# amathislab/myochallenge

Measured on AMD Instinct MI355X. Metric: env-steps/sec (Baoding, 4096 envs), higher is better.
Workload: dtype f64

## Files before the change

### myochallenge_amd/csrc/myo_ppo_mlp.h

```cpp
#pragma once
#ifndef MYO_EMU
#include "myo_act.h"

typedef __attribute__((ext_vector_type(8))) __bf16 myo_bf16x8;
typedef __attribute__((ext_vector_type(4))) float myo_f32x4;

#define MLP_H 256
#define MLP_OPMAX 128
#define MLP_APM 48
#define MLP_AKP 64
#define MLP_XS (MLP_OPMAX + 8)
#define MLP_HS (MLP_H + 8)
#define MLP_DS (MLP_AKP + 8)
#define MLP_SOS 49
#define MLP_SPLITK 16

struct MlpImages { unsigned short *W1p, *W2, *W2T, *Whp, *WhT; float* bias; };
static inline MlpImages mlp_images_carve(unsigned char* base, int OP, size_t* bytes) {
  size_t o = 0;
  auto take = [&](size_t n) { unsigned char* p = base ? base + o : nullptr; o += (n + 255) / 256 * 256; return p; };
  const size_t H = MLP_H;
  MlpImages w;
  w.W1p = (unsigned short*)take(2 * H * OP * 2); w.W2 = (unsigned short*)take(2 * H * H * 2); w.W2T = (unsigned short*)take(2 * H * H * 2);
  w.Whp = (unsigned short*)take(2 * MLP_APM * H * 2); w.WhT = (unsigned short*)take(2 * H * MLP_AKP * 2);
// ... 114 lines not shown
  if (t == 0) { part[3 * blockIdx.x] = (float)n; part[3 * blockIdx.x + 1] = mean; part[3 * blockIdx.x + 2] = (red[0] + red[1]) + (red[2] + red[3]); }
}
__global__ void __launch_bounds__(256) k_adv_merge(const float* __restrict__ part_all, int nb, int B, float* __restrict__ stats) {
  __shared__ float sp[3 * MLP_ADV_BLOCKS];
  const int t = threadIdx.x;
  if (t < 3 * nb) sp[t] = part_all[(size_t)blockIdx.x * 3 * nb + t];
  __syncthreads();
  if (t == 0) mlp_adv_merge(sp, nb, B, stats + 2 * blockIdx.x);
}

struct MlpImgTarget {
  MlpImages img;
  int off_W1[2], off_b1[2], off_W2[2], off_b2[2], off_Wh[2], off_bh[2];
  int O, OP, A;
};
__device__ __forceinline__ void mlp_img_store(const MlpImgTarget& T, int i, float x) {
  constexpr unsigned H = MLP_H;
#pragma unroll
  for (int net = 0; net < 2; ++net) {
    const unsigned Ah = net == 0 ? (unsigned)T.A : 1u;
    unsigned j = (unsigned)(i - T.off_W2[net]);
    if (j < H * H) {
      const unsigned short v = mlp_f2bf(x);
      T.img.W2[net * H * H + j] = v;
      T.img.W2T[net * H * H + (j % H) * H + j / H] = v;
      return;
    }
    j = (unsigned)(i - T.off_W1[net]);
    if (j < H * (unsigned)T.O) { const unsigned o = j / (unsigned)T.O; T.img.W1p[net * H * T.OP + o * T.OP + (j - o * T.O)] = mlp_f2bf(x); return; }
    j = (unsigned)(i - T.off_Wh[net]);
    if (j < Ah * H) {
      const unsigned short v = mlp_f2bf(x);
      T.img.Whp[net * MLP_APM * H + j] = v;
      T.img.WhT[net * H * MLP_AKP + (j % H) * MLP_AKP + j / H] = v;
      return;
    }
    j = (unsigned)(i - T.off_b1[net]);
    if (j < H) { T.img.bias[net * H + j] = x; return; }
    j = (unsigned)(i - T.off_b2[net]);
    if (j < H) { T.img.bias[2 * H + net * H + j] = x; return; }
    j = (unsigned)(i - T.off_bh[net]);
    if (j < Ah) { T.img.bias[4 * H + net * MLP_APM + j] = x; return; }
  }
}

template <int KSTEPS>
__device__ __forceinline__ void mlp_load_w(myo_bf16x8 (&bw)[8][4], const unsigned short* Wg, int w_stride, int n0, int lm, int lq) {
#pragma unroll
  for (int ks = 0; ks < KSTEPS; ++ks)
#pragma unroll
    for (int nt = 0; nt < 4; ++nt) bw[ks][nt] = *reinterpret_cast<const myo_bf16x8*>(Wg + (size_t)(n0 + 16 * nt + lm) * w_stride + 32 * ks + 8 * lq);
  __builtin_amdgcn_sched_barrier(0);
}
template <int KSTEPS, int MT>
__device__ __forceinline__ void mlp_mma_slab(myo_f32x4 (&acc)[MT][4], const unsigned short* As, int as_stride, const myo_bf16x8 (&bw)[8][4],
                                             int lm, int lq) {
#pragma unroll
  for (int mt = 0; mt < MT; ++mt)
#pragma unroll
    for (int nt = 0; nt < 4; ++nt) acc[mt][nt] = myo_f32x4{0.f, 0.f, 0.f, 0.f};
#pragma unroll
  for (int ks = 0; ks < KSTEPS; ++ks) {
#pragma unroll
    for (int m2 = 0; m2 < MT; m2 += 2) {
      myo_bf16x8 a[2];
#pragma unroll
      for (int mt = 0; mt < 2; ++mt) a[mt] = *reinterpret_cast<const myo_bf16x8*>(As + (16 * (m2 + mt) + lm) * as_stride + 32 * ks + 8 * lq);
#pragma unroll
      for (int mt = 0; mt < 2; ++mt)
#pragma unroll
        for (int nt = 0; nt < 4; ++nt) acc[m2 + mt][nt] = __builtin_amdgcn_mfma_f32_16x16x32_bf16(a[mt], bw[ks][nt], acc[m2 + mt][nt], 0, 0, 0);
    }
  }
  __builtin_amdgcn_sched_barrier(0);
}

#ifdef MLP_PROF
__device__ unsigned long long g_mlp_prof[16];
#ifndef MLP_PROF_NET
#define MLP_PROF_NET 0
#endif
#define MLP_STAMP(k) { __syncthreads(); if (threadIdx.x == 0 && blockIdx.x == 3 && blockIdx.y == MLP_PROF_NET) g_mlp_prof[k] = wall_clock64(); }
extern "C" int myo_debug_mlp_prof(unsigned long long* out) { return (int)hipMemcpyFromSymbol(out, HIP_SYMBOL(g_mlp_prof), sizeof g_mlp_prof); }
#else
#define MLP_STAMP(k)
#endif

#ifndef MLP_BM
#define MLP_BM 32
#endif
#define MLP_FWDBWD_LDS (512 + MLP_BM * MLP_XS * 2 + MLP_BM * MLP_HS * 2 + MLP_BM * MLP_SOS * 4 + MLP_BM * MLP_DS * 2 + 128 * 4 + 192 * 4)

template <int ACT>
__device__ __forceinline__ float mlp_act(float x) { return ACT == MYO_ACT_TANH ? myo_act_tanh(x) : fmaxf(x, 0.f); }

template <int MT>
__device__ __forceinline__ void mlp_store_act_tanh(const myo_f32x4 (&acc)[MT][4], const float (&bb)[4], unsigned short* Hs, unsigned short* HT,
                                                   size_t B, int r0, int n0, int lm, int lq) {
#pragma unroll
  for (int mt = 0; mt < MT; ++mt)
#pragma unroll
    for (int nt = 0; nt < 4; ++nt) {
      const int n = n0 + 16 * nt + lm, m = 16 * mt + 4 * lq;
      unsigned short h[4];
#pragma unroll
      for (int r = 0; r < 4; ++r) { h[r] = mlp_f2bf(mlp_act<MYO_ACT_TANH>(acc[mt][nt][r] + bb[nt])); Hs[(m + r) * MLP_HS + n] = h[r]; }
      *reinterpret_cast<uint2*>(HT + (size_t)n * B + r0 + m) = make_uint2((unsigned)h[0] | ((unsigned)h[1] << 16), (unsigned)h[2] | ((unsigned)h[3] << 16));
    }
}
template <int MT>
__device__ __forceinline__ void mlp_load_act(uint2 (&hv)[MT][4], const unsigned short* HT, size_t B, int r0, int n0, int lm, int lq) {
#pragma unroll
  for (int mt = 0; mt < MT; ++mt)
#pragma unroll
    for (int nt = 0; nt < 4; ++nt) hv[mt][nt] = *reinterpret_cast<const uint2*>(HT + (size_t)(n0 + 16 * nt + lm) * B + r0 + 16 * mt + 4 * lq);
  __builtin_amdgcn_sched_barrier(0);
}
template <int MT, bool TO_LDS>
__device__ __forceinline__ void mlp_store_grad_tanh(const myo_f32x4 (&acc)[MT][4], const uint2 (&hv)[MT][4], unsigned short* Hs, unsigned short* HT,
                                                    size_t B, int r0, int n0, int lm, int lq) {
#pragma unroll
  for (int mt = 0; mt < MT; ++mt)
#pragma unroll
    for (int nt = 0; nt < 4; ++nt) {
      const int n = n0 + 16 * nt + lm, m = 16 * mt + 4 * lq;
      const float hf[4] = {__uint_as_float(hv[mt][nt].x << 16), __uint_as_float(hv[mt][nt].x & 0xffff0000u),
                           __uint_as_float(hv[mt][nt].y << 16), __uint_as_float(hv[mt][nt].y & 0xffff0000u)};
      unsigned short h[4];
#pragma unroll
      for (int r = 0; r < 4; ++r) {
        h[r] = mlp_f2bf(mlp_bf2f(mlp_f2bf(acc[mt][nt][r])) * fmaf(-hf[r], hf[r], 1.f));
        if (TO_LDS) Hs[(m + r) * MLP_HS + n] = h[r];
      }
      *reinterpret_cast<uint2*>(HT + (size_t)n * B + r0 + m) = make_uint2((unsigned)h[0] | ((unsigned)h[1] << 16), (unsigned)h[2] | ((unsigned)h[3] << 16));
    }
}

template <int MT>
__device__ __forceinline__ unsigned long long mlp_store_act(const myo_f32x4 (&acc)[MT][4], const float (&bb)[4], unsigned short* Hs, unsigned short* HT,
                                                            size_t B, int r0, int n0, int lm, int lq) {
  static_assert(MT * 16 <= 64, "one mask bit per accumulator element");
  unsigned long long mask = 0;
#pragma unroll
  for (int mt = 0; mt < MT; ++mt)
#pragma unroll
    for (int nt = 0; nt < 4; ++nt) {
      const int n = n0 + 16 * nt + lm, m = 16 * mt + 4 * lq;
      unsigned short h[4];
#pragma unroll
      for (int r = 0; r < 4; ++r) {
        h[r] = mlp_f2bf(fmaxf(acc[mt][nt][r] + bb[nt], 0.f)); Hs[(m + r) * MLP_HS + n] = h[r];
        mask |= (unsigned long long)(h[r] != 0) << (16 * mt + 4 * nt + r);
      }
      *reinterpret_cast<uint2*>(HT + (size_t)n * B + r0 + m) = make_uint2((unsigned)h[0] | ((unsigned)h[1] << 16), (unsigned)h[2] | ((unsigned)h[3] << 16));
    }
  return mask;
}
template <int MT, bool TO_LDS>
__device__ __forceinline__ void mlp_store_grad(const myo_f32x4 (&acc)[MT][4], unsigned long long mask, unsigned short* Hs, unsigned short* HT, size_t B,
                                               int r0, int n0, int lm, int lq) {
#pragma unroll
  for (int mt = 0; mt < MT; ++mt)
#pragma unroll
    for (int nt = 0; nt < 4; ++nt) {
      const int n = n0 + 16 * nt + lm, m = 16 * mt + 4 * lq;
      unsigned short h[4];
#pragma unroll
      for (int r = 0; r < 4; ++r) {
        const unsigned short on = (unsigned short)(-(int)((mask >> (16 * mt + 4 * nt + r)) & 1ull));
        h[r] = mlp_f2bf(acc[mt][nt][r]) & on;
        if (TO_LDS) Hs[(m + r) * MLP_HS + n] = h[r];
      }
      *reinterpret_cast<uint2*>(HT + (size_t)n * B + r0 + m) = make_uint2((unsigned)h[0] | ((unsigned)h[1] << 16), (unsigned)h[2] | ((unsigned)h[3] << 16));
    }
}

template <int ACT>
__global__ void __launch_bounds__(256, 2) k_mlp_fwdbwd(MlpArgs P) {
  constexpr int H = MLP_H, XS = MLP_XS, HS = MLP_HS, DS = MLP_DS, SOS = MLP_SOS, BM = MLP_BM, MT = BM / 16, RW = BM / 4;
  extern __shared__ __align__(16) unsigned char mlp_smem[];
  long long* s_idx = reinterpret_cast<long long*>(mlp_smem);
  unsigned short* Xs = reinterpret_cast<unsigned short*>(mlp_smem + 512);
  float* So = reinterpret_cast<float*>(mlp_smem + 512);
  unsigned short* Hs = Xs + BM * XS;
  float* Sa = reinterpret_cast<float*>(Hs + BM * HS);
  unsigned short* dOs = reinterpret_cast<unsigned short*>(Sa + BM * SOS);
  float* s_ls = reinterpret_cast<float*>(dOs + BM * DS);
  float* s_row = s_ls + 128;
  static_assert(BM * MLP_SOS * 4 <= BM * MLP_XS * 2, "the head output tile fits where X was");
  static_assert(BM == 32 || BM == 64, "wave / tile mapping below");
  const int t = threadIdx.x, w = t >> 6, lane = t & 63, lm = lane & 15, lq = lane >> 4;
  const int net = blockIdx.y, blk = blockIdx.x, r0 = blk * BM, B = P.B, O = P.O, A = P.A, OP = P.OP;
  const int n0 = 64 * w;
  MLP_STAMP(0)
  if (t < BM) s_idx[t] = P.idx[r0 + t];
  if (t < A) { const float ls = P.log_std[t]; s_ls[t] = ls; s_ls[64 + t] = __expf(-ls); }
  const float* b1 = P.img.bias + net * H; const float* b2 = P.img.bias + 2 * H + net * H; const float* bh = P.img.bias + 4 * H + net * MLP_APM;
  float bb1[4], bb2[4];
#pragma unroll
  for (int nt = 0; nt < 4; ++nt) { bb1[nt] = b1[n0 + 16 * nt + lm]; bb2[nt] = b2[n0 + 16 * nt + lm]; }
  myo_bf16x8 bw[8][4];
  {
    const unsigned short* W1 = P.img.W1p + (size_t)net * H * OP;
    if (OP == 96) mlp_load_w<3>(bw, W1, OP, n0, lm, lq);
    else if (OP == 128) mlp_load_w<4>(bw, W1, OP, n0, lm, lq);
    else if (OP == 64) mlp_load_w<2>(bw, W1, OP, n0, lm, lq);
    else mlp_load_w<1>(bw, W1, OP, n0, lm, lq);
  }
  __syncthreads();
  if (t < BM) {
    const size_t src = (size_t)s_idx[t];
    s_row[t] = P.adv[src]; s_row[64 + t] = P.oldlp[src]; s_row[128 + t] = P.ret[src];
  }
  {
    float v[RW][2], av[RW];
#pragma unroll
    for (int k = 0; k < RW; ++k) {
      const size_t row = (size_t)s_idx[RW * w + k];
      v[k][0] = lane < O ? P.obs[row * O + lane] : 0.f;
      v[k][1] = lane + 64 < O ? P.obs[row * O + lane + 64] : 0.f;
      av[k] = (net == 0 && lane < A) ? P.act[row * A + lane] : 0.f;
    }
#pragma unroll
    for (int k = 0; k < RW; ++k) {
      Xs[(RW * w + k) * XS + lane] = mlp_f2bf(v[k][0]);
      if (lane + 64 < OP) Xs[(RW * w + k) * XS + lane + 64] = mlp_f2bf(v[k][1]);
      if (lane < A) Sa[(RW * w + k) * SOS + lane] = av[k];
    }
    if (net == 0) {
#pragma unroll
      for (int h = 0; h < 2; ++h) {
        const int c = lane + 64 * h;
        if (c < OP) {
          unsigned u[RW / 2];
#pragma unroll
          for (int k = 0; k < RW / 2; ++k) u[k] = (unsigned)mlp_f2bf(v[2 * k][h]) | ((unsigned)mlp_f2bf(v[2 * k + 1][h]) << 16);
          uint4* dst = reinterpret_cast<uint4*>(P.XT + (size_t)c * B + r0 + RW * w);
#pragma unroll
          for (int q = 0; q < RW / 8; ++q) dst[q] = make_uint4(u[4 * q], u[4 * q + 1], u[4 * q + 2], u[4 * q + 3]);
        }
      }
    }
  }
  __syncthreads();
  MLP_STAMP(1)
  myo_f32x4 acc[MT][4];
  if (OP == 96) mlp_mma_slab<3, MT>(acc, Xs, XS, bw, lm, lq);
  else if (OP == 128) mlp_mma_slab<4, MT>(acc, Xs, XS, bw, lm, lq);
  else if (OP == 64) mlp_mma_slab<2, MT>(acc, Xs, XS, bw, lm, lq);
  else mlp_mma_slab<1, MT>(acc, Xs, XS, bw, lm, lq);
  mlp_load_w<H / 32>(bw, P.img.W2 + (size_t)net * H * H, H, n0, lm, lq);
  unsigned long long mask1 = 0, mask2 = 0;
  if (ACT == MYO_ACT_TANH) mlp_store_act_tanh<MT>(acc, bb1, Hs, P.H1T + (size_t)net * H * B, B, r0, n0, lm, lq);
  else mask1 = mlp_store_act<MT>(acc, bb1, Hs, P.H1T + (size_t)net * H * B, B, r0, n0, lm, lq);
  __syncthreads();
  MLP_STAMP(2)
  mlp_mma_slab<H / 32, MT>(acc, Hs, HS, bw, lm, lq);
  const unsigned short* Wh = P.img.Whp + (size_t)net * MLP_APM * H;
  myo_bf16x8 bh2[H / 32];
  if (w < 3) {
#pragma unroll
    for (int ks = 0; ks < H / 32; ++ks) bh2[ks] = *reinterpret_cast<const myo_bf16x8*>(Wh + (size_t)(16 * w + lm) * H + 32 * ks + 8 * lq);
  }
  __builtin_amdgcn_sched_barrier(0);
  __syncthreads();
  if (ACT == MYO_ACT_TANH) mlp_store_act_tanh<MT>(acc, bb2, Hs, P.H2T + (size_t)net * H * B, B, r0, n0, lm, lq);
  else mask2 = mlp_store_act<MT>(acc, bb2, Hs, P.H2T + (size_t)net * H * B, B, r0, n0, lm, lq);
  __syncthreads();
  MLP_STAMP(3)
  if (w < 3) {
    const float bv = bh[16 * w + lm];
#pragma unroll
    for (int mt = 0; mt < MT; ++mt) {
      myo_f32x4 ah = myo_f32x4{0.f, 0.f, 0.f, 0.f};
#pragma unroll
      for (int ks = 0; ks < H / 32; ++ks) {
        const myo_bf16x8 a = *reinterpret_cast<const myo_bf16x8*>(Hs + (16 * mt + lm) * HS + 32 * ks + 8 * lq);
        ah = __builtin_amdgcn_mfma_f32_16x16x32_bf16(a, bh2[ks], ah, 0, 0, 0);
      }
#pragma unroll
      for (int r = 0; r < 4; ++r) So[(16 * mt + 4 * lq + r) * SOS + 16 * w + lm] = ah[r] + bv;
    }
  }
  mlp_load_w<MLP_AKP / 32>(bw, P.img.WhT + (size_t)net * H * MLP_AKP, MLP_AKP, n0, lm, lq);
  __syncthreads();
  MLP_STAMP(4)
  const int NB = P.NB;
  if (w == 0) {
    const int r = lane < BM ? lane : 0;
    const bool on = lane < BM;
    if (net == 0) {
      float logp = 0.f;
      for (int a = 0; a < A; ++a) {
        const float z = (Sa[r * SOS + a] - So[r * SOS + a]) * s_ls[64 + a];
        logp += -0.5f * z * z - s_ls[a] - 0.9189385332046727f;
      }
      const float an = (s_row[r] - P.adv_stats[0]) / (P.adv_stats[1] + 1e-8f);
      const float clip = P.hp ? P.hp[MYO_HP_CLIP] : P.clip;
      const float lr_i = logp - s_row[64 + r];
      const float ratio = __expf(lr_i);
      const float s1 = an * ratio;
      const float rc = fminf(fmaxf(ratio, 1.f - clip), 1.f + clip);
      const float s2 = an * rc;
      float pl_i = on ? -fminf(s1, s2) / B : 0.f;
      const bool inside = (ratio > 1.f - clip) && (ratio < 1.f + clip);
      const float dlogp = -(an * ratio) * ((s1 <= s2) ? 1.f : (inside ? 1.f : 0.f)) / B;
      if (on) {
        for (int a = 0; a < A; ++a) {
          const float inv = s_ls[64 + a];
          const float z = (Sa[r * SOS + a] - So[r * SOS + a]) * inv;
          const float dm = dlogp * z * inv;
          So[r * SOS + a] = dm;
          Sa[r * SOS + a] = dlogp * (z * z - 1.f);
          dOs[r * DS + a] = mlp_f2bf(dm);
        }
        for (int a = A; a < MLP_AKP; ++a) dOs[r * DS + a] = 0;
      }
      for (int off = 32; off >= 1; off >>= 1) pl_i += __shfl_xor(pl_i, off, 64);
      if (lane == 0) P.part[(size_t)A * NB + blk] = pl_i;
      if (P.hp) {
        float ent = 0.f;
        for (int a = 0; a < A; ++a) ent += s_ls[a] + 1.4189385332046727f;
        float kl_i = on ? ((ratio - 1.f) - lr_i) / B : 0.f, cf_i = on ? (fabsf(ratio - 1.f) > clip ? 1.f : 0.f) / B : 0.f;
        float el_i = on ? -ent / B : 0.f;
        for (int off = 32; off >= 1; off >>= 1) {
          kl_i += __shfl_xor(kl_i, off, 64); cf_i += __shfl_xor(cf_i, off, 64); el_i += __shfl_xor(el_i, off, 64);
        }
        if (lane == 0) {
          P.part[(size_t)(2 * A + 3) * NB + blk] = kl_i; P.part[(size_t)(2 * A + 4) * NB + blk] = cf_i;
          P.part[(size_t)(2 * A + 5) * NB + blk] = el_i;
        }
      }
    } else {
      const float dv = So[r * SOS] - s_row[128 + r];
      float vl_i = on ? dv * dv / B : 0.f, dv_i = on ? P.vf_coef * 2.f / B * dv : 0.f;
      if (on) {
        dOs[r * DS] = mlp_f2bf(dv_i);
        for (int a = 1; a < MLP_AKP; ++a) dOs[r * DS + a] = 0;
      }
      for (int off = 32; off >= 1; off >>= 1) { vl_i += __shfl_xor(vl_i, off, 64); dv_i += __shfl_xor(dv_i, off, 64); }
      if (lane == 0) { P.part[(size_t)(A + 1) * NB + blk] = vl_i; P.part[(size_t)(2 * A + 2) * NB + blk] = dv_i; }
    }
  }
  __syncthreads();
  MLP_STAMP(5)
  if (net == 0 && t < A) {
    float my_ls = 0.f, my_db = 0.f;
    for (int r = 0; r < BM; ++r) { my_ls += Sa[r * SOS + t]; my_db += So[r * SOS + t]; }
    P.part[(size_t)t * NB + blk] = my_ls; P.part[(size_t)(A + 2 + t) * NB + blk] = my_db;
  }
  {
    const int Ah = net == 0 ? A : 1;
    for (int e = t; e < Ah * (BM / 8); e += 256) {
      const int c = e / (BM / 8), ch = e % (BM / 8);
      unsigned v[4];
#pragma unroll
      for (int k = 0; k < 4; ++k) v[k] = (unsigned)dOs[(8 * ch + 2 * k) * DS + c] | ((unsigned)dOs[(8 * ch + 2 * k + 1) * DS + c] << 16);
      *reinterpret_cast<uint4*>(P.dOT + ((size_t)net * 128 + c) * B + r0 + 8 * ch) = make_uint4(v[0], v[1], v[2], v[3]);
    }
  }
  MLP_STAMP(6)
  uint2 hv[MT][4];
  if (ACT == MYO_ACT_TANH) mlp_load_act<MT>(hv, P.H2T + (size_t)net * H * B, B, r0, n0, lm, lq);
  mlp_mma_slab<MLP_AKP / 32, MT>(acc, dOs, DS, bw, lm, lq);
  mlp_load_w<H / 32>(bw, P.img.W2T + (size_t)net * H * H, H, n0, lm, lq);
  if (ACT == MYO_ACT_TANH) {
    mlp_store_grad_tanh<MT, true>(acc, hv, Hs, P.dH2T + (size_t)net * H * B, B, r0, n0, lm, lq);
    mlp_load_act<MT>(hv, P.H1T + (size_t)net * H * B, B, r0, n0, lm, lq);
  } else {
    mlp_store_grad<MT, true>(acc, mask2, Hs, P.dH2T + (size_t)net * H * B, B, r0, n0, lm, lq);
  }
  __syncthreads();
  MLP_STAMP(7)
  mlp_mma_slab<H / 32, MT>(acc, Hs, HS, bw, lm, lq);
  if (ACT == MYO_ACT_TANH) mlp_store_grad_tanh<MT, false>(acc, hv, Hs, P.dH1T + (size_t)net * H * B, B, r0, n0, lm, lq);
  else mlp_store_grad<MT, false>(acc, mask1, Hs, P.dH1T + (size_t)net * H * B, B, r0, n0, lm, lq);
  MLP_STAMP(8)
}

struct MlpPolicyArgs {
  const float* obs;
  const float* log_std;
  MlpImages img;
  float* obs_buf;
  float *act_buf, *val_buf, *logp_buf, *clipped;
  const int* t_idx;
  unsigned long long* draw_counter;
  unsigned long long seed;
  int N, O, A, OP, deterministic;
};
#define MLP_POLICY_LDS (MLP_BM * MLP_XS * 2 + MLP_BM * MLP_HS * 2 + 128 * 4)

template <int ACT, int MT>
__device__ __forceinline__ void mlp_store_act_lds(const myo_f32x4 (&acc)[MT][4], const float (&bb)[4], unsigned short* Hs, int n0, int lm, int lq) {
#pragma unroll
  for (int mt = 0; mt < MT; ++mt)
#pragma unroll
    for (int nt = 0; nt < 4; ++nt) {
      const int n = n0 + 16 * nt + lm, m = 16 * mt + 4 * lq;
#pragma unroll
      for (int r = 0; r < 4; ++r) Hs[(m + r) * MLP_HS + n] = mlp_f2bf(mlp_act<ACT>(acc[mt][nt][r] + bb[nt]));
    }
}

template <int ACT>
__global__ void __launch_bounds__(256, 2) k_mlp_policy(MlpPolicyArgs P) {
  constexpr int H = MLP_H, XS = MLP_XS, HS = MLP_HS, SOS = MLP_SOS, BM = MLP_BM, MT = BM / 16, RW = BM / 4;
  extern __shared__ __align__(16) unsigned char mlp_smem[];
  unsigned short* Xs = reinterpret_cast<unsigned short*>(mlp_smem);
  float* So = reinterpret_cast<float*>(mlp_smem);
  unsigned short* Hs = Xs + BM * XS;
  float* s_ls = reinterpret_cast<float*>(Hs + BM * HS);
  static_assert(BM * MLP_SOS * 4 <= BM * MLP_XS * 2, "the head output tile fits where X was");
  const int t = threadIdx.x, w = t >> 6, lane = t & 63, lm = lane & 15, lq = lane >> 4;
  const int net = blockIdx.y, r0 = blockIdx.x * BM, N = P.N, O = P.O, A = P.A, OP = P.OP;
  const int n0 = 64 * w;
  const size_t tt = (size_t)(*P.t_idx);
  if (t < A) { const float ls = P.log_std[t]; s_ls[t] = ls; s_ls[64 + t] = __expf(ls); }
  const float* b1 = P.img.bias + net * H; const float* b2 = P.img.bias + 2 * H + net * H; const float* bh = P.img.bias + 4 * H + net * MLP_APM;
  float bb1[4], bb2[4];
#pragma unroll
  for (int nt = 0; nt < 4; ++nt) { bb1[nt] = b1[n0 + 16 * nt + lm]; bb2[nt] = b2[n0 + 16 * nt + lm]; }
  myo_bf16x8 bw[8][4];
  {
    const unsigned short* W1 = P.img.W1p + (size_t)net * H * OP;
    if (OP == 96) mlp_load_w<3>(bw, W1, OP, n0, lm, lq);
    else if (OP == 128) mlp_load_w<4>(bw, W1, OP, n0, lm, lq);
    else if (OP == 64) mlp_load_w<2>(bw, W1, OP, n0, lm, lq);
    else mlp_load_w<1>(bw, W1, OP, n0, lm, lq);
  }
// ... 235 lines not shown
```

### myochallenge_amd/csrc/myobatch.hip

```cpp
#include <hip/hip_runtime.h>
#include <utility>
#include <vector>
#define MYO_BACKEND_NAME "gfx950"
#define MYO_BACKEND_DENSE_NEWTON 0
#define MYO_BACKEND_BATCH_FIELDS hipEvent_t ev0, ev1; std::vector<std::pair<hipEvent_t, hipEvent_t>> pending;
#define MYO_BACKEND_RENDER_ENVS_MAX 65535
struct DeviceGuard {
  int prev = -1; bool switched = false;
  explicit DeviceGuard(int dev) { if (hipGetDevice(&prev) == hipSuccess && prev != dev) switched = (hipSetDevice(dev) == hipSuccess); }
  ~DeviceGuard() { if (switched) (void)hipSetDevice(prev); }
};
#include "myo_host.h"

static int be_malloc(void** p, size_t n) { return (int)hipMalloc(p, n ? n : 1); }
static void be_free(void* p) { (void)hipFree(p); }
static int be_h2d(void* d, const void* h, size_t n) { return (int)hipMemcpy(d, h, n, hipMemcpyHostToDevice); }
static int be_set_device(int dev) { return (int)hipSetDevice(dev); }
static const char* be_errstr(int e) { return hipGetErrorString((hipError_t)e); }

#define MYO_MAX_DEVICES 64
struct BoundDev { const myo_batch* b = nullptr; hipStream_t last = nullptr; bool have_last = false; hipEvent_t ev = nullptr; };
static BoundDev g_bound[MYO_MAX_DEVICES];
static std::mutex g_bound_mu;
struct SlotWs { double* p = nullptr; int* map = nullptr; int users = 0; char* big = nullptr; int big_users = 0; };
// ... 1575 lines not shown
  return hidden == MLP_H && O >= 1 && O <= MLP_OPMAX && A >= 1 && A <= MLP_APM && B >= 64 * MLP_SPLITK && B % (64 * MLP_SPLITK) == 0;
}
static int mlp_shape_check(const myo_ppo_mlp_desc* d, const char* who) {
  if (mlp_shape_ok(d->B, d->O, d->A, d->hidden)) return MYO_OK;
  return fail(MYO_E_UNSUPPORTED, "%s: needs hidden = %d, obs <= %d, act <= %d, batch a multiple of %d", who, MLP_H, MLP_OPMAX, MLP_APM, 64 * MLP_SPLITK);
}
extern "C" long long myo_ppo_mlp_workspace_bytes(int B, int obs_dim, int act_dim, int hidden, long long G) {
  if (!mlp_shape_ok(B, obs_dim, act_dim, hidden) || G <= 0) return -1;
  return (long long)mlp_carve(nullptr, B, (obs_dim + 31) / 32 * 32, act_dim, G).bytes;
}
extern "C" int myo_ppo_mlp_sqnorm_parts(int act_dim) {
  return MLP_RF_BLOCKS + 2 * act_dim + 3;
}
static void mlp_launch_prep(const float* p, const myo_mlp_layout& lay, int O, int A, const MlpImages& img, const float* adv_part, float* adv_stats,
                            int adv_nb, int B, hipStream_t st) {
  MlpPrepArgs pp;
  pp.p = p; pp.O = O; pp.OP = (O + 31) / 32 * 32; pp.Ah[0] = A; pp.Ah[1] = 1; pp.img = img;
  for (int k = 0; k < 2; ++k) {
    pp.off_W1[k] = lay.off_W1[k]; pp.off_b1[k] = lay.off_b1[k]; pp.off_W2[k] = lay.off_W2[k]; pp.off_b2[k] = lay.off_b2[k];
    pp.off_Wh[k] = lay.off_Wh[k]; pp.off_bh[k] = lay.off_bh[k];
  }
  pp.adv_part = adv_part; pp.adv_stats = adv_stats; pp.adv_nb = adv_nb; pp.B = B;
  hipLaunchKernelGGL(k_mlp_prep, dim3(256), dim3(256), 0, st, pp);
}
static int mlp_step(const myo_ppo_mlp_desc* d, void* stream, bool resident, int activation, const char* who) {
  if (!d || !d->obs || !d->act || !d->oldlp || !d->adv || !d->ret || !d->idx || !d->params || !d->grads || !d->adv_stats || !d->acc ||
      !d->workspace)
    return fail(MYO_E_ARG, "%s: null argument", who);
  if (!myo_act_known(activation)) return fail(MYO_E_ARG, "%s: unknown activation code %d", who, activation);
  const int B = d->B, O = d->O, A = d->A, OP = (O + 31) / 32 * 32;
  const myo_mlp_layout& lay = d->layout;
  if (int rc = mlp_shape_check(d, who)) return rc;
  if (resident && d->compute_adv_stats) return fail(MYO_E_ARG, "%s: the advantage moments are the caller's (compute_adv_stats = 0)", who);
  const MlpWs w = mlp_carve((unsigned char*)d->workspace, B, OP, A, d->G);
  if ((long long)w.bytes > d->workspace_bytes) return fail(MYO_E_ARG, "%s: workspace too small (%zu bytes needed)", who, w.bytes);
  hipStream_t st = (hipStream_t)stream;
  const bool tanh_act = activation == MYO_ACT_TANH;
  void (*const fwdbwd)(MlpArgs) = tanh_act ? k_mlp_fwdbwd<MYO_ACT_TANH> : k_mlp_fwdbwd<MYO_ACT_RELU>;
  static bool lds_set[2] = {false, false};
  if (!lds_set[tanh_act]) {
    if (hipFuncSetAttribute((const void*)fwdbwd, hipFuncAttributeMaxDynamicSharedMemorySize, MLP_FWDBWD_LDS) != hipSuccess)
      return fail(MYO_E_DEVICE, "%s: cannot reserve %d bytes of LDS", who, (int)MLP_FWDBWD_LDS);
    lds_set[tanh_act] = true;
  }
  if (!resident) {
    if (d->compute_adv_stats) hipLaunchKernelGGL(k_adv_moments, dim3(MLP_ADV_BLOCKS), dim3(256), 0, st, d->adv, (const long long*)d->idx, B, w.advpart);
    mlp_launch_prep(d->params, lay, O, A, w.img, w.advpart, d->adv_stats, d->compute_adv_stats ? MLP_ADV_BLOCKS : 0, B, st);
  }
  MlpArgs a;
  a.obs = d->obs; a.act = d->act; a.oldlp = d->oldlp; a.adv = d->adv; a.ret = d->ret; a.idx = (const long long*)d->idx;
  a.log_std = d->params + lay.off_log_std; a.adv_stats = d->adv_stats; a.img = w.img;
  a.XT = w.XT; a.H1T = w.H1T; a.H2T = w.H2T; a.dH1T = w.dH1T; a.dH2T = w.dH2T; a.dOT = w.dOT; a.part = w.part;
  a.B = B; a.O = O; a.A = A; a.OP = OP; a.NB = B / MLP_BM; a.clip = d->clip; a.vf_coef = d->vf_coef; a.hp = d->hp;
  hipLaunchKernelGGL(fwdbwd, dim3(B / MLP_BM, 2), dim3(256), MLP_FWDBWD_LDS, st, a);
  MlpWgradArgs g;
  g.njobs = 0; g.B = B; g.rows_per_split = B / MLP_SPLITK; g.G = d->G; g.slab = w.slab;
  const size_t HB = (size_t)MLP_H * B;
  for (int net = 0; net < 2; ++net) {
    for (int m0 = 0; m0 < MLP_H; m0 += 128) {
      for (int n0 = 0; n0 < MLP_H; n0 += 128)
        g.job[g.njobs++] = MlpWgradJob{w.dH2T + net * HB, w.H1T + net * HB, MLP_H, MLP_H, MLP_H, m0, n0, lay.off_W2[net], n0 == 0 ? lay.off_b2[net] : -1};
      g.job[g.njobs++] = MlpWgradJob{w.dH1T + net * HB, w.XT, MLP_H, O, O, m0, 0, lay.off_W1[net], lay.off_b1[net]};
    }
    for (int n0 = 0; n0 < MLP_H; n0 += 128)
      g.job[g.njobs++] = MlpWgradJob{w.dOT + (size_t)net * 128 * B, w.H2T + net * HB, net == 0 ? A : 1, MLP_H, MLP_H, 0, n0, lay.off_Wh[net], -1};
  }
  hipLaunchKernelGGL(k_mlp_wgrad, dim3(g.njobs * MLP_SPLITK), dim3(256), 0, st, g);
  if (d->sqnorm_part && d->adam_step) {
    MlpRfArgs rf;
    rf.slab = w.slab; rf.g = d->grads; rf.G = d->G; rf.splits = MLP_SPLITK; rf.part = w.part; rf.acc = d->acc; rf.NB = B / MLP_BM; rf.A = A;
    rf.ent_coef = d->ent_coef; rf.off_log_std = lay.off_log_std; rf.off_bh0 = lay.off_bh[0]; rf.off_bh1 = lay.off_bh[1];
    rf.sq_part = d->sqnorm_part; rf.adam_step = d->adam_step; rf.hp = d->hp;
    hipLaunchKernelGGL(k_mlp_reduce_finish, dim3(MLP_RF_BLOCKS + 2 * A + 3), dim3(256), 0, st, rf);
  } else {
    hipLaunchKernelGGL(k_mlp_reduce, dim3((unsigned)((d->G + 255) / 256)), dim3(256), 0, st, (const float*)w.slab, d->grads, d->G, MLP_SPLITK);
    hipLaunchKernelGGL(k_colmajor_finish, dim3(2 * A + 3 + (d->hp ? 1 : 0)), dim3(64), 0, st, (const float*)w.part, d->acc, B / MLP_BM, A, d->ent_coef,
                       d->grads + lay.off_log_std, d->grads + lay.off_bh[0], d->grads + lay.off_bh[1], d->hp);
  }
  LAUNCH_CHECK(0)
  return MYO_OK;
}
extern "C" int myo_ppo_mlp_step_act(const myo_ppo_mlp_desc* d, int resident, int activation, void* stream) {
  return mlp_step(d, stream, resident != 0, activation, "myo_ppo_mlp_step_act");
}
extern "C" int myo_ppo_mlp_step(const myo_ppo_mlp_desc* d, void* stream) { return mlp_step(d, stream, false, MYO_ACT_RELU, "myo_ppo_mlp_step"); }
extern "C" int myo_ppo_mlp_step_resident(const myo_ppo_mlp_desc* d, void* stream) { return mlp_step(d, stream, true, MYO_ACT_RELU, "myo_ppo_mlp_step_resident"); }
static int mlp_images_ok(const myo_ppo_mlp_desc* d, const char* who, MlpImages* img) {
  if (!d || !d->params || !d->workspace) return fail(MYO_E_ARG, "%s: null argument", who);
  if (int rc = mlp_shape_check(d, who)) return rc;
  const MlpWs w = mlp_carve((unsigned char*)d->workspace, d->B, (d->O + 31) / 32 * 32, d->A, d->G);
  if ((long long)w.bytes > d->workspace_bytes) return fail(MYO_E_ARG, "%s: workspace too small (%zu bytes needed)", who, w.bytes);
  *img = w.img;
  return MYO_OK;
}
extern "C" int myo_ppo_mlp_images(const myo_ppo_mlp_desc* d, void* stream) {
  MlpImages img;
  if (int rc = mlp_images_ok(d, "myo_ppo_mlp_images", &img)) return rc;
  mlp_launch_prep(d->params, d->layout, d->O, d->A, img, nullptr, nullptr, 0, d->B, (hipStream_t)stream);
  LAUNCH_CHECK(0)
  return MYO_OK;
}

static int mlp_img_target(const myo_ppo_mlp_desc* d, int n, const char* who, MlpImgTarget* T) {
  if (int rc = mlp_images_ok(d, who, &T->img)) return rc;
  if (d->G != n) return fail(MYO_E_ARG, "%s: the descriptor's parameter vector has %lld elements, this one %d", who, (long long)d->G, n);
  bool inside = true;
  auto put = [&](int (&dst)[2], const int64_t (&src)[2]) {
// ... 179 lines not shown
```

Baseline: 1.757 million.

## Process both actor and critic nets in one fwd/bwd block sharing staged inputs

The fused MLP forward/backward kernel no longer launches a second grid dimension for the two networks. Each block now gathers and stages the observation/action rows once, then runs the actor pass and the critic pass back to back with a lambda. This removes the duplicated index gather, observation load and LDS staging for the critic, and halves the block count. The cost is a longer serial chain per block, less parallelism, and a larger LDS footprint because the head-output tile now gets its own buffer instead of aliasing X, which could reduce occupancy.

```diff
diff --git a/myochallenge_amd/csrc/myo_ppo_mlp.h b/myochallenge_amd/csrc/myo_ppo_mlp.h
--- a/myochallenge_amd/csrc/myo_ppo_mlp.h
+++ b/myochallenge_amd/csrc/myo_ppo_mlp.h
@@ -190,6 +190,12 @@
     for (int nt = 0; nt < 4; ++nt) bw[ks][nt] = *reinterpret_cast<const myo_bf16x8*>(Wg + (size_t)(n0 + 16 * nt + lm) * w_stride + 32 * ks + 8 * lq);
   __builtin_amdgcn_sched_barrier(0);
 }
+__device__ __forceinline__ void mlp_load_w1(myo_bf16x8 (&bw)[8][4], const unsigned short* W1, int OP, int n0, int lm, int lq) {
+  if (OP == 96) mlp_load_w<3>(bw, W1, OP, n0, lm, lq);
+  else if (OP == 128) mlp_load_w<4>(bw, W1, OP, n0, lm, lq);
+  else if (OP == 64) mlp_load_w<2>(bw, W1, OP, n0, lm, lq);
+  else mlp_load_w<1>(bw, W1, OP, n0, lm, lq);
+}
 template <int KSTEPS, int MT>
 __device__ __forceinline__ void mlp_mma_slab(myo_f32x4 (&acc)[MT][4], const unsigned short* As, int as_stride, const myo_bf16x8 (&bw)[8][4],
                                              int lm, int lq) {
@@ -215,10 +221,7 @@
 
 #ifdef MLP_PROF
 __device__ unsigned long long g_mlp_prof[16];
-#ifndef MLP_PROF_NET
-#define MLP_PROF_NET 0
-#endif
-#define MLP_STAMP(k) { __syncthreads(); if (threadIdx.x == 0 && blockIdx.x == 3 && blockIdx.y == MLP_PROF_NET) g_mlp_prof[k] = wall_clock64(); }
+#define MLP_STAMP(k) { __syncthreads(); if (threadIdx.x == 0 && blockIdx.x == 3) g_mlp_prof[k] = wall_clock64(); }
 extern "C" int myo_debug_mlp_prof(unsigned long long* out) { return (int)hipMemcpyFromSymbol(out, HIP_SYMBOL(g_mlp_prof), sizeof g_mlp_prof); }
 #else
 #define MLP_STAMP(k)
@@ -227,7 +230,7 @@
 #ifndef MLP_BM
 #define MLP_BM 32
 #endif
-#define MLP_FWDBWD_LDS (512 + MLP_BM * MLP_XS * 2 + MLP_BM * MLP_HS * 2 + MLP_BM * MLP_SOS * 4 + MLP_BM * MLP_DS * 2 + 128 * 4 + 192 * 4)
+#define MLP_FWDBWD_LDS (512 + MLP_BM * MLP_XS * 2 + MLP_BM * MLP_HS * 2 + 2 * MLP_BM * MLP_SOS * 4 + MLP_BM * MLP_DS * 2 + 128 * 4 + 192 * 4)
 
 template <int ACT>
 __device__ __forceinline__ float mlp_act(float x) { return ACT == MYO_ACT_TANH ? myo_act_tanh(x) : fmaxf(x, 0.f); }
@@ -319,32 +322,21 @@
   extern __shared__ __align__(16) unsigned char mlp_smem[];
   long long* s_idx = reinterpret_cast<long long*>(mlp_smem);
   unsigned short* Xs = reinterpret_cast<unsigned short*>(mlp_smem + 512);
-  float* So = reinterpret_cast<float*>(mlp_smem + 512);
   unsigned short* Hs = Xs + BM * XS;
   float* Sa = reinterpret_cast<float*>(Hs + BM * HS);
   unsigned short* dOs = reinterpret_cast<unsigned short*>(Sa + BM * SOS);
   float* s_ls = reinterpret_cast<float*>(dOs + BM * DS);
   float* s_row = s_ls + 128;
-  static_assert(BM * MLP_SOS * 4 <= BM * MLP_XS * 2, "the head output tile fits where X was");
+  float* So = s_row + 192;
   static_assert(BM == 32 || BM == 64, "wave / tile mapping below");
-  const int t = threadIdx.x, w = t >> 6, lane = t & 63, lm = lane & 15, lq = lane >> 4;
-  const int net = blockIdx.y, blk = blockIdx.x, r0 = blk * BM, B = P.B, O = P.O, A = P.A, OP = P.OP;
-  const int n0 = 64 * w;
+  const int t = threadIdx.x, w = t >> 6, lane = t & 63, lm_o = lane & 15, lq_o = lane >> 4;
+  const int blk = blockIdx.x, r0 = blk * BM, B = P.B, O = P.O, A = P.A, OP = P.OP;
+  const int n0_o = 64 * w;
   MLP_STAMP(0)
   if (t < BM) s_idx[t] = P.idx[r0 + t];
   if (t < A) { const float ls = P.log_std[t]; s_ls[t] = ls; s_ls[64 + t] = __expf(-ls); }
-  const float* b1 = P.img.bias + net * H; const float* b2 = P.img.bias + 2 * H + net * H; const float* bh = P.img.bias + 4 * H + net * MLP_APM;
-  float bb1[4], bb2[4];
-#pragma unroll
-  for (int nt = 0; nt < 4; ++nt) { bb1[nt] = b1[n0 + 16 * nt + lm]; bb2[nt] = b2[n0 + 16 * nt + lm]; }
   myo_bf16x8 bw[8][4];
-  {
-    const unsigned short* W1 = P.img.W1p + (size_t)net * H * OP;
-    if (OP == 96) mlp_load_w<3>(bw, W1, OP, n0, lm, lq);
-    else if (OP == 128) mlp_load_w<4>(bw, W1, OP, n0, lm, lq);
-    else if (OP == 64) mlp_load_w<2>(bw, W1, OP, n0, lm, lq);
-    else mlp_load_w<1>(bw, W1, OP, n0, lm, lq);
-  }
+  mlp_load_w1(bw, P.img.W1p, OP, n0_o, lm_o, lq_o);
   __syncthreads();
   if (t < BM) {
     const size_t src = (size_t)s_idx[t];
@@ -357,7 +349,7 @@
       const size_t row = (size_t)s_idx[RW * w + k];
       v[k][0] = lane < O ? P.obs[row * O + lane] : 0.f;
       v[k][1] = lane + 64 < O ? P.obs[row * O + lane + 64] : 0.f;
-      av[k] = (net == 0 && lane < A) ? P.act[row * A + lane] : 0.f;
+      av[k] = lane < A ? P.act[row * A + lane] : 0.f;
     }
 #pragma unroll
     for (int k = 0; k < RW; ++k) {
@@ -365,155 +357,165 @@
       if (lane + 64 < OP) Xs[(RW * w + k) * XS + lane + 64] = mlp_f2bf(v[k][1]);
       if (lane < A) Sa[(RW * w + k) * SOS + lane] = av[k];
     }
-    if (net == 0) {
-#pragma unroll
-      for (int h = 0; h < 2; ++h) {
-        const int c = lane + 64 * h;
-        if (c < OP) {
-          unsigned u[RW / 2];
-#pragma unroll
-          for (int k = 0; k < RW / 2; ++k) u[k] = (unsigned)mlp_f2bf(v[2 * k][h]) | ((unsigned)mlp_f2bf(v[2 * k + 1][h]) << 16);
-          uint4* dst = reinterpret_cast<uint4*>(P.XT + (size_t)c * B + r0 + RW * w);
-#pragma unroll
-          for (int q = 0; q < RW / 8; ++q) dst[q] = make_uint4(u[4 * q], u[4 * q + 1], u[4 * q + 2], u[4 * q + 3]);
+#pragma unroll
+    for (int h = 0; h < 2; ++h) {
+      const int c = lane + 64 * h;
+      if (c < OP) {
+        unsigned u[RW / 2];
+#pragma unroll
+        for (int k = 0; k < RW / 2; ++k) u[k] = (unsigned)mlp_f2bf(v[2 * k][h]) | ((unsigned)mlp_f2bf(v[2 * k + 1][h]) << 16);
+        uint4* dst = reinterpret_cast<uint4*>(P.XT + (size_t)c * B + r0 + RW * w);
+#pragma unroll
+        for (int q = 0; q < RW / 8; ++q) dst[q] = make_uint4(u[4 * q], u[4 * q + 1], u[4 * q + 2], u[4 * q + 3]);
+      }
+    }
+  }
+  __syncthreads();
+  MLP_STAMP(1)
+  const int NB = P.NB;
+  auto pass = [&](const int net) __attribute__((always_inline)) {
+    int lm = lm_o, lq = lq_o, n0 = n0_o;
+    asm volatile("" : "+v"(lm), "+v"(lq), "+v"(n0));
+    if (net == 1) mlp_load_w1(bw, P.img.W1p + (size_t)H * OP, OP, n0, lm, lq);
+    const float* b1 = P.img.bias + net * H; const float* b2 = P.img.bias + 2 * H + net * H; const float* bh = P.img.bias + 4 * H + net * MLP_APM;
+    float bb1[4], bb2[4];
+#pragma unroll
+    for (int nt = 0; nt < 4; ++nt) { bb1[nt] = b1[n0 + 16 * nt + lm]; bb2[nt] = b2[n0 + 16 * nt + lm]; }
+    myo_f32x4 acc[MT][4];
+    if (OP == 96) mlp_mma_slab<3, MT>(acc, Xs, XS, bw, lm, lq);
+    else if (OP == 128) mlp_mma_slab<4, MT>(acc, Xs, XS, bw, lm, lq);
+    else if (OP == 64) mlp_mma_slab<2, MT>(acc, Xs, XS, bw, lm, lq);
+    else mlp_mma_slab<1, MT>(acc, Xs, XS, bw, lm, lq);
+    mlp_load_w<H / 32>(bw, P.img.W2 + (size_t)net * H * H, H, n0, lm, lq);
+    unsigned long long mask1 = 0, mask2 = 0;
+    if (ACT == MYO_ACT_TANH) mlp_store_act_tanh<MT>(acc, bb1, Hs, P.H1T + (size_t)net * H * B, B, r0, n0, lm, lq);
+    else mask1 = mlp_store_act<MT>(acc, bb1, Hs, P.H1T + (size_t)net * H * B, B, r0, n0, lm, lq);
+    __syncthreads();
+    MLP_STAMP(7 * net + 2)
+    mlp_mma_slab<H / 32, MT>(acc, Hs, HS, bw, lm, lq);
+    const unsigned short* Wh = P.img.Whp + (size_t)net * MLP_APM * H;
+    myo_bf16x8 bh2[H / 32];
+    if (w < 3) {
+#pragma unroll
+      for (int ks = 0; ks < H / 32; ++ks) bh2[ks] = *reinterpret_cast<const myo_bf16x8*>(Wh + (size_t)(16 * w + lm) * H + 32 * ks + 8 * lq);
+    }
+    __builtin_amdgcn_sched_barrier(0);
+    __syncthreads();
+    if (ACT == MYO_ACT_TANH) mlp_store_act_tanh<MT>(acc, bb2, Hs, P.H2T + (size_t)net * H * B, B, r0, n0, lm, lq);
+    else mask2 = mlp_store_act<MT>(acc, bb2, Hs, P.H2T + (size_t)net * H * B, B, r0, n0, lm, lq);
+    __syncthreads();
+    MLP_STAMP(7 * net + 3)
+    if (w < 3) {
+      const float bv = bh[16 * w + lm];
+#pragma unroll
+      for (int mt = 0; mt < MT; ++mt) {
+        myo_f32x4 ah = myo_f32x4{0.f, 0.f, 0.f, 0.f};
+#pragma unroll
+        for (int ks = 0; ks < H / 32; ++ks) {
+          const myo_bf16x8 a = *reinterpret_cast<const myo_bf16x8*>(Hs + (16 * mt + lm) * HS + 32 * ks + 8 * lq);
+          ah = __builtin_amdgcn_mfma_f32_16x16x32_bf16(a, bh2[ks], ah, 0, 0, 0);
         }
-      }
-    }
-  }
-  __syncthreads();
-  MLP_STAMP(1)
-  myo_f32x4 acc[MT][4];
-  if (OP == 96) mlp_mma_slab<3, MT>(acc, Xs, XS, bw, lm, lq);
-  else if (OP == 128) mlp_mma_slab<4, MT>(acc, Xs, XS, bw, lm, lq);
-  else if (OP == 64) mlp_mma_slab<2, MT>(acc, Xs, XS, bw, lm, lq);
-  else mlp_mma_slab<1, MT>(acc, Xs, XS, bw, lm, lq);
-  mlp_load_w<H / 32>(bw, P.img.W2 + (size_t)net * H * H, H, n0, lm, lq);
-  unsigned long long mask1 = 0, mask2 = 0;
-  if (ACT == MYO_ACT_TANH) mlp_store_act_tanh<MT>(acc, bb1, Hs, P.H1T + (size_t)net * H * B, B, r0, n0, lm, lq);
-  else mask1 = mlp_store_act<MT>(acc, bb1, Hs, P.H1T + (size_t)net * H * B, B, r0, n0, lm, lq);
-  __syncthreads();
-  MLP_STAMP(2)
-  mlp_mma_slab<H / 32, MT>(acc, Hs, HS, bw, lm, lq);
-  const unsigned short* Wh = P.img.Whp + (size_t)net * MLP_APM * H;
-  myo_bf16x8 bh2[H / 32];
-  if (w < 3) {
-#pragma unroll
-    for (int ks = 0; ks < H / 32; ++ks) bh2[ks] = *reinterpret_cast<const myo_bf16x8*>(Wh + (size_t)(16 * w + lm) * H + 32 * ks + 8 * lq);
-  }
-  __builtin_amdgcn_sched_barrier(0);
-  __syncthreads();
-  if (ACT == MYO_ACT_TANH) mlp_store_act_tanh<MT>(acc, bb2, Hs, P.H2T + (size_t)net * H * B, B, r0, n0, lm, lq);
-  else mask2 = mlp_store_act<MT>(acc, bb2, Hs, P.H2T + (size_t)net * H * B, B, r0, n0, lm, lq);
-  __syncthreads();
-  MLP_STAMP(3)
-  if (w < 3) {
-    const float bv = bh[16 * w + lm];
-#pragma unroll
-    for (int mt = 0; mt < MT; ++mt) {
-      myo_f32x4 ah = myo_f32x4{0.f, 0.f, 0.f, 0.f};
-#pragma unroll
-      for (int ks = 0; ks < H / 32; ++ks) {
-        const myo_bf16x8 a = *reinterpret_cast<const myo_bf16x8*>(Hs + (16 * mt + lm) * HS + 32 * ks + 8 * lq);
-        ah = __builtin_amdgcn_mfma_f32_16x16x32_bf16(a, bh2[ks], ah, 0, 0, 0);
-      }
-#pragma unroll
-      for (int r = 0; r < 4; ++r) So[(16 * mt + 4 * lq + r) * SOS + 16 * w + lm] = ah[r] + bv;
-    }
-  }
-  mlp_load_w<MLP_AKP / 32>(bw, P.img.WhT + (size_t)net * H * MLP_AKP, MLP_AKP, n0, lm, lq);
-  __syncthreads();
-  MLP_STAMP(4)
-  const int NB = P.NB;
-  if (w == 0) {
-    const int r = lane < BM ? lane : 0;
-    const bool on = lane < BM;
-    if (net == 0) {
-      float logp = 0.f;
-      for (int a = 0; a < A; ++a) {
-        const float z = (Sa[r * SOS + a] - So[r * SOS + a]) * s_ls[64 + a];
-        logp += -0.5f * z * z - s_ls[a] - 0.9189385332046727f;
-      }
-      const float an = (s_row[r] - P.adv_stats[0]) / (P.adv_stats[1] + 1e-8f);
-      const float clip = P.hp ? P.hp[MYO_HP_CLIP] : P.clip;
-      const float lr_i = logp - s_row[64 + r];
-      const float ratio = __expf(lr_i);
-      const float s1 = an * ratio;
-      const float rc = fminf(fmaxf(ratio, 1.f - clip), 1.f + clip);
-      const float s2 = an * rc;
-      float pl_i = on ? -fminf(s1, s2) / B : 0.f;
-      const bool inside = (ratio > 1.f - clip) && (ratio < 1.f + clip);
-      const float dlogp = -(an * ratio) * ((s1 <= s2) ? 1.f : (inside ? 1.f : 0.f)) / B;
-      if (on) {
+#pragma unroll
+        for (int r = 0; r < 4; ++r) So[(16 * mt + 4 * lq + r) * SOS + 16 * w + lm] = ah[r] + bv;
+      }
+    }
+    mlp_load_w<MLP_AKP / 32>(bw, P.img.WhT + (size_t)net * H * MLP_AKP, MLP_AKP, n0, lm, lq);
+    __syncthreads();
+    MLP_STAMP(7 * net + 4)
+    if (w == 0) {
+      const int r = lane < BM ? lane : 0;
+      const bool on = lane < BM;
+      if (net == 0) {
+        float logp = 0.f;
         for (int a = 0; a < A; ++a) {
-          const float inv = s_ls[64 + a];
-          const float z = (Sa[r * SOS + a] - So[r * SOS + a]) * inv;
-          const float dm = dlogp * z * inv;
-          So[r * SOS + a] = dm;
-          Sa[r * SOS + a] = dlogp * (z * z - 1.f);
-          dOs[r * DS + a] = mlp_f2bf(dm);
+          const float z = (Sa[r * SOS + a] - So[r * SOS + a]) * s_ls[64 + a];
+          logp += -0.5f * z * z - s_ls[a] - 0.9189385332046727f;
         }
-        for (int a = A; a < MLP_AKP; ++a) dOs[r * DS + a] = 0;
-      }
-      for (int off = 32; off >= 1; off >>= 1) pl_i += __shfl_xor(pl_i, off, 64);
-      if (lane == 0) P.part[(size_t)A * NB + blk] = pl_i;
-      if (P.hp) {
-        float ent = 0.f;
-        for (int a = 0; a < A; ++a) ent += s_ls[a] + 1.4189385332046727f;
-        float kl_i = on ? ((ratio - 1.f) - lr_i) / B : 0.f, cf_i = on ? (fabsf(ratio - 1.f) > clip ? 1.f : 0.f) / B : 0.f;
-        float el_i = on ? -ent / B : 0.f;
-        for (int off = 32; off >= 1; off >>= 1) {
-          kl_i += __shfl_xor(kl_i, off, 64); cf_i += __shfl_xor(cf_i, off, 64); el_i += __shfl_xor(el_i, off, 64);
+        const float an = (s_row[r] - P.adv_stats[0]) / (P.adv_stats[1] + 1e-8f);
+        const float clip = P.hp ? P.hp[MYO_HP_CLIP] : P.clip;
+        const float lr_i = logp - s_row[64 + r];
+        const float ratio = __expf(lr_i);
+        const float s1 = an * ratio;
+        const float rc = fminf(fmaxf(ratio, 1.f - clip), 1.f + clip);
+        const float s2 = an * rc;
+        float pl_i = on ? -fminf(s1, s2) / B : 0.f;
+        const bool inside = (ratio > 1.f - clip) && (ratio < 1.f + clip);
+        const float dlogp = -(an * ratio) * ((s1 <= s2) ? 1.f : (inside ? 1.f : 0.f)) / B;
+        if (on) {
+          for (int a = 0; a < A; ++a) {
+            const float inv = s_ls[64 + a];
+            const float z = (Sa[r * SOS + a] - So[r * SOS + a]) * inv;
+            const float dm = dlogp * z * inv;
+            So[r * SOS + a] = dm;
+            Sa[r * SOS + a] = dlogp * (z * z - 1.f);
+            dOs[r * DS + a] = mlp_f2bf(dm);
+          }
+          for (int a = A; a < MLP_AKP; ++a) dOs[r * DS + a] = 0;
         }
-        if (lane == 0) {
-          P.part[(size_t)(2 * A + 3) * NB + blk] = kl_i; P.part[(size_t)(2 * A + 4) * NB + blk] = cf_i;
-          P.part[(size_t)(2 * A + 5) * NB + blk] = el_i;
+        for (int off = 32; off >= 1; off >>= 1) pl_i += __shfl_xor(pl_i, off, 64);
+        if (lane == 0) P.part[(size_t)A * NB + blk] = pl_i;
+        if (P.hp) {
+          float ent = 0.f;
+          for (int a = 0; a < A; ++a) ent += s_ls[a] + 1.4189385332046727f;
+          float kl_i = on ? ((ratio - 1.f) - lr_i) / B : 0.f, cf_i = on ? (fabsf(ratio - 1.f) > clip ? 1.f : 0.f) / B : 0.f;
+          float el_i = on ? -ent / B : 0.f;
+          for (int off = 32; off >= 1; off >>= 1) {
+            kl_i += __shfl_xor(kl_i, off, 64); cf_i += __shfl_xor(cf_i, off, 64); el_i += __shfl_xor(el_i, off, 64);
+          }
+          if (lane == 0) {
+            P.part[(size_t)(2 * A + 3) * NB + blk] = kl_i; P.part[(size_t)(2 * A + 4) * NB + blk] = cf_i;
+            P.part[(size_t)(2 * A + 5) * NB + blk] = el_i;
+          }
         }
-      }
+      } else {
+        const float dv = So[r * SOS] - s_row[128 + r];
+        float vl_i = on ? dv * dv / B : 0.f, dv_i = on ? P.vf_coef * 2.f / B * dv : 0.f;
+        if (on) {
+          dOs[r * DS] = mlp_f2bf(dv_i);
+          for (int a = 1; a < MLP_AKP; ++a) dOs[r * DS + a] = 0;
+        }
+        for (int off = 32; off >= 1; off >>= 1) { vl_i += __shfl_xor(vl_i, off, 64); dv_i += __shfl_xor(dv_i, off, 64); }
+        if (lane == 0) { P.part[(size_t)(A + 1) * NB + blk] = vl_i; P.part[(size_t)(2 * A + 2) * NB + blk] = dv_i; }
+      }
+    }
+    __syncthreads();
+    MLP_STAMP(7 * net + 5)
+    if (net == 0 && t < A) {
+      float my_ls = 0.f, my_db = 0.f;
+      for (int r = 0; r < BM; ++r) { my_ls += Sa[r * SOS + t]; my_db += So[r * SOS + t]; }
+      P.part[(size_t)t * NB + blk] = my_ls; P.part[(size_t)(A + 2 + t) * NB + blk] = my_db;
+    }
+    {
+      const int Ah = net == 0 ? A : 1;
+      for (int e = t; e < Ah * (BM / 8); e += 256) {
+        const int c = e / (BM / 8), ch = e % (BM / 8);
+        unsigned v[4];
+#pragma unroll
+        for (int k = 0; k < 4; ++k) v[k] = (unsigned)dOs[(8 * ch + 2 * k) * DS + c] | ((unsigned)dOs[(8 * ch + 2 * k + 1) * DS + c] << 16);
+        *reinterpret_cast<uint4*>(P.dOT + ((size_t)net * 128 + c) * B + r0 + 8 * ch) = make_uint4(v[0], v[1], v[2], v[3]);
+      }
+    }
+    MLP_STAMP(7 * net + 6)
+    uint2 hv[MT][4];
+    if (ACT == MYO_ACT_TANH) mlp_load_act<MT>(hv, P.H2T + (size_t)net * H * B, B, r0, n0, lm, lq);
+    mlp_mma_slab<MLP_AKP / 32, MT>(acc, dOs, DS, bw, lm, lq);
+    mlp_load_w<H / 32>(bw, P.img.W2T + (size_t)net * H * H, H, n0, lm, lq);
+    if (ACT == MYO_ACT_TANH) {
+      mlp_store_grad_tanh<MT, true>(acc, hv, Hs, P.dH2T + (size_t)net * H * B, B, r0, n0, lm, lq);
+      mlp_load_act<MT>(hv, P.H1T + (size_t)net * H * B, B, r0, n0, lm, lq);
     } else {
-      const float dv = So[r * SOS] - s_row[128 + r];
-      float vl_i = on ? dv * dv / B : 0.f, dv_i = on ? P.vf_coef * 2.f / B * dv : 0.f;
-      if (on) {
-        dOs[r * DS] = mlp_f2bf(dv_i);
-        for (int a = 1; a < MLP_AKP; ++a) dOs[r * DS + a] = 0;
-      }
-      for (int off = 32; off >= 1; off >>= 1) { vl_i += __shfl_xor(vl_i, off, 64); dv_i += __shfl_xor(dv_i, off, 64); }
-      if (lane == 0) { P.part[(size_t)(A + 1) * NB + blk] = vl_i; P.part[(size_t)(2 * A + 2) * NB + blk] = dv_i; }
-    }
-  }
-  __syncthreads();
-  MLP_STAMP(5)
-  if (net == 0 && t < A) {
-    float my_ls = 0.f, my_db = 0.f;
-    for (int r = 0; r < BM; ++r) { my_ls += Sa[r * SOS + t]; my_db += So[r * SOS + t]; }
-    P.part[(size_t)t * NB + blk] = my_ls; P.part[(size_t)(A + 2 + t) * NB + blk] = my_db;
-  }
-  {
-    const int Ah = net == 0 ? A : 1;
-    for (int e = t; e < Ah * (BM / 8); e += 256) {
-      const int c = e / (BM / 8), ch = e % (BM / 8);
-      unsigned v[4];
-#pragma unroll
-      for (int k = 0; k < 4; ++k) v[k] = (unsigned)dOs[(8 * ch + 2 * k) * DS + c] | ((unsigned)dOs[(8 * ch + 2 * k + 1) * DS + c] << 16);
-      *reinterpret_cast<uint4*>(P.dOT + ((size_t)net * 128 + c) * B + r0 + 8 * ch) = make_uint4(v[0], v[1], v[2], v[3]);
-    }
-  }
-  MLP_STAMP(6)
-  uint2 hv[MT][4];
-  if (ACT == MYO_ACT_TANH) mlp_load_act<MT>(hv, P.H2T + (size_t)net * H * B, B, r0, n0, lm, lq);
-  mlp_mma_slab<MLP_AKP / 32, MT>(acc, dOs, DS, bw, lm, lq);
-  mlp_load_w<H / 32>(bw, P.img.W2T + (size_t)net * H * H, H, n0, lm, lq);
-  if (ACT == MYO_ACT_TANH) {
-    mlp_store_grad_tanh<MT, true>(acc, hv, Hs, P.dH2T + (size_t)net * H * B, B, r0, n0, lm, lq);
-    mlp_load_act<MT>(hv, P.H1T + (size_t)net * H * B, B, r0, n0, lm, lq);
-  } else {
-    mlp_store_grad<MT, true>(acc, mask2, Hs, P.dH2T + (size_t)net * H * B, B, r0, n0, lm, lq);
-  }
-  __syncthreads();
-  MLP_STAMP(7)
-  mlp_mma_slab<H / 32, MT>(acc, Hs, HS, bw, lm, lq);
-  if (ACT == MYO_ACT_TANH) mlp_store_grad_tanh<MT, false>(acc, hv, Hs, P.dH1T + (size_t)net * H * B, B, r0, n0, lm, lq);
-  else mlp_store_grad<MT, false>(acc, mask1, Hs, P.dH1T + (size_t)net * H * B, B, r0, n0, lm, lq);
-  MLP_STAMP(8)
+      mlp_store_grad<MT, true>(acc, mask2, Hs, P.dH2T + (size_t)net * H * B, B, r0, n0, lm, lq);
+    }
+    __syncthreads();
+    MLP_STAMP(7 * net + 7)
+    mlp_mma_slab<H / 32, MT>(acc, Hs, HS, bw, lm, lq);
+    if (ACT == MYO_ACT_TANH) mlp_store_grad_tanh<MT, false>(acc, hv, Hs, P.dH1T + (size_t)net * H * B, B, r0, n0, lm, lq);
+    else mlp_store_grad<MT, false>(acc, mask1, Hs, P.dH1T + (size_t)net * H * B, B, r0, n0, lm, lq);
+    __syncthreads();
+    MLP_STAMP(7 * net + 8)
+  };
+  pass(0);
+  pass(1);
 }
 
 struct MlpPolicyArgs {
diff --git a/myochallenge_amd/csrc/myobatch.hip b/myochallenge_amd/csrc/myobatch.hip
--- a/myochallenge_amd/csrc/myobatch.hip
+++ b/myochallenge_amd/csrc/myobatch.hip
@@ -1651,7 +1651,7 @@
   a.log_std = d->params + lay.off_log_std; a.adv_stats = d->adv_stats; a.img = w.img;
   a.XT = w.XT; a.H1T = w.H1T; a.H2T = w.H2T; a.dH1T = w.dH1T; a.dH2T = w.dH2T; a.dOT = w.dOT; a.part = w.part;
   a.B = B; a.O = O; a.A = A; a.OP = OP; a.NB = B / MLP_BM; a.clip = d->clip; a.vf_coef = d->vf_coef; a.hp = d->hp;
-  hipLaunchKernelGGL(fwdbwd, dim3(B / MLP_BM, 2), dim3(256), MLP_FWDBWD_LDS, st, a);
+  hipLaunchKernelGGL(fwdbwd, dim3(B / MLP_BM), dim3(256), MLP_FWDBWD_LDS, st, a);
   MlpWgradArgs g;
   g.njobs = 0; g.B = B; g.rows_per_split = B / MLP_SPLITK; g.G = d->G; g.slab = w.slab;
   const size_t HB = (size_t)MLP_H * B;
```

Result: no change. 1.774 million, median of 6 (+0.9%).
